# nicoloalbergoni/DeepLabV3Plus-Augmented-SuperResolution

Measured on AMD Instinct MI355X. Metric: augmented-copies/sec (fwd+realign+SR-iter) @512x512, higher is better.
Workload: dtype f32 (pointwise GEMMs: operands split into f16 hi+lo, hi*hi+hi*lo+lo*hi on f16 MFMA, f32 accumulate)

## Files before the change

__graft_entry__.py:

```python
from __future__ import annotations

import importlib.util
import os
import sys

ROOT = os.path.dirname(os.path.abspath(__file__))
if ROOT not in sys.path:
    sys.path.insert(0, ROOT)

PKG_DIR = os.path.join(ROOT, "deeplabv3plus-augmented-superresolution_amd")


def _load_build_module():
    spec = importlib.util.spec_from_file_location("asr_csrc_build", os.path.join(PKG_DIR, "csrc", "build.py"))
    mod = importlib.util.module_from_spec(spec)
    spec.loader.exec_module(mod)
    return mod


def build() -> None:
    lib = _load_build_module().build(force=False, verbose=True)
    assert os.path.exists(lib), lib
    import asr_amd
    asr_amd._lib.load()
    import asr_amd.ops
    print(f"built and loaded {lib} (ABI v{asr_amd._lib.load().asr_abi_version()})")


def smoke() -> None:
    import numpy as np
    import torch

    build()
    assert torch.cuda.is_available(), "smoke() needs a GPU"
    torch.cuda.set_device(0)
    dev = torch.device("cuda", 0)
    from asr_amd import ops, weights as W
    from asr_amd.model import DeeplabModel
    from asr_amd.pipeline import HotPath
    from asr_amd.superresolution_scripts.optimizer import Optimizer
    from asr_amd.superresolution_scripts.superresolution import Superresolution
    from asr_amd.superresolution_scripts.augmentation_utils import draw_augmentation_parameters
    from oracle import augment as o_aug, sr as o_sr
    from oracle.model import OracleDeeplabV3Plus

    size, feat, n_aug, iters, cls = (128, 128), (32, 32), 4, 5, 8
    weights = W.make_synthetic_weights(1234, 21)
    import bench
    img = bench.synth_image(np.random.default_rng(7), size[0])
    np.random.seed(1234)
    angles, shifts = draw_augmentation_parameters(n_aug, 0.15, 20)

    model = DeeplabModel(weights, size + (3,), 21, final_upsample=False, last_activation=None)
    img_dev = ops.to_device(img, device=dev)
    weights = bench.shifted_weights(weights, cls, bench.calibrate_class_bias(model, img_dev, cls))
# ... 41 lines not shown
```

deeplabv3plus-augmented-superresolution_amd/csrc/build.py:

```python
from __future__ import annotations

import os
import subprocess
import sys

HERE = os.path.dirname(os.path.abspath(__file__))
PKG = os.path.dirname(HERE)
LIB = os.path.join(PKG, "libasr_hip.so")
VARIANTS = {"phase": ["-DASR_GEMM_PHASE_PROFILE"],
            "diag": []}
VARIANT_SOURCES = {"diag": [(os.path.join("diag", "gemm_diag.hip"), [])]}

NO_PK_F32 = ["-Xclang", "-target-feature", "-Xclang", "-packed-fp32-ops"]
_HOST_NOISE = "'-packed-fp32-ops' is not a recognized feature for this target"

SOURCES = [
    ("core.cpp", []),
    ("warp.hip", ["-ffp-contract=off"] + NO_PK_F32),
    ("sr.hip", ["-ffp-contract=off"]),
    ("reduce.hip", ["-ffp-contract=off"] + NO_PK_F32),
    ("gemm.hip", ["-Wno-inline-asm"] + NO_PK_F32),
    ("dwconv.hip", NO_PK_F32),
    ("layers.hip", NO_PK_F32),
    ("sepconv.hip", NO_PK_F32),
# ... 31 lines not shown
    return any(os.path.getmtime(d) > t for d in deps)


def _postpass(hipcc, flags, src, obj, verbose):
    import importlib.util
    spec = importlib.util.spec_from_file_location("asr_pk_postpass", os.path.join(HERE, "pk_postpass.py"))
    pp = importlib.util.module_from_spec(spec)
    spec.loader.exec_module(pp)
    if not os.path.exists(os.path.join(pp.LLVM, "clang-offload-bundler")):
        print(f"build.py: no LLVM tools under {pp.LLVM}: {os.path.basename(src)} is built without packed-f32", file=sys.stderr, flush=True)
        return False
    try:
        n = pp.compile_with_postpass(hipcc, flags, src, obj)
    except pp.Unsafe as e:
        print(f"build.py: post-pass cannot split `{e}`: {os.path.basename(src)} is built without packed-f32", file=sys.stderr, flush=True)
        return False
    if verbose:
        print(f"{hipcc} ... {os.path.basename(src)} (packed-f32 post-pass: {n} op_sel:[0,1] instructions split)", flush=True)
    return True


def _isa_guard(lib):
    import importlib.util
    spec = importlib.util.spec_from_file_location("asr_isa_guard", os.path.join(HERE, "isa_guard.py"))
    guard = importlib.util.module_from_spec(spec)
    spec.loader.exec_module(guard)
    try:
        return guard.violations(lib)
    except guard.ToolMissing as e:
        print(f"build.py: isa_guard skipped ({e})", file=sys.stderr, flush=True)
        return []


def build(force=False, verbose=True):
    import fcntl
    variant = os.environ.get("ASR_BUILD_VARIANT", "")
    if variant and variant not in VARIANTS:
        raise ValueError(f"ASR_BUILD_VARIANT must be one of {sorted(VARIANTS)} (got {variant!r})")
    objdir = os.path.join(HERE, "build_" + variant if variant else "build")
    os.makedirs(objdir, exist_ok=True)
    with open(os.path.join(objdir, ".lock"), "w") as lock:
        fcntl.flock(lock, fcntl.LOCK_EX)
        try:
            return _build_locked(objdir, force, verbose, variant)
        finally:
            fcntl.flock(lock, fcntl.LOCK_UN)


def _build_locked(objdir, force, verbose, variant=""):
    hipcc = _hipcc()
    lib = os.path.join(PKG, f"libasr_hip_{variant}.so") if variant else LIB
    extra_all = VARIANTS.get(variant, []) + os.environ.get("ASR_EXTRA_HIPFLAGS", "").split()
    stamp = os.path.join(objdir, "flags.txt")
    flags_now = " ".join(COMMON + extra_all)
    if not os.path.exists(stamp) or open(stamp).read() != flags_now:
        force = True
    hdrs = [os.path.join(HERE, h) for h in HEADERS] + [os.path.abspath(__file__)]
    objs = []
    for src, extra in ALL_SOURCES + VARIANT_SOURCES.get(variant, []):
        s = os.path.join(HERE, src)
        o = os.path.join(objdir, os.path.splitext(os.path.basename(src))[0] + ".o")
        objs.append(o)
        if force or _stale(o, [s] + hdrs + ([os.path.join(HERE, "pk_postpass.py")] if src in POSTPASS else [])):
            if src in POSTPASS and _postpass(hipcc, COMMON + extra + extra_all, s, o, verbose):
                continue
            if src in POSTPASS:
                extra = extra + NO_PK_F32
            cmd = [hipcc] + COMMON + extra + extra_all + ["-c", s, "-o", o]
            if verbose:
                print(" ".join(cmd), flush=True)
            _compile(cmd)
    relinked = force or _stale(lib, objs)
    if relinked:
        cmd = [hipcc, "--offload-arch=gfx950", "-shared", "-fPIC", "-o", lib] + objs
        if verbose:
            print(" ".join(cmd), flush=True)
        subprocess.check_call(cmd)
    with open(stamp, "w") as fh:
        fh.write(flags_now)
    if relinked and not variant:
        bad = _isa_guard(lib)
        if bad:
            os.replace(lib, lib + ".rejected")
            raise RuntimeError("isa_guard: %d violation(s) in the product library, first: %s in %s (%s); kept as %s"
                               % (len(bad), bad[0][1], bad[0][0], bad[0][2], lib + ".rejected"))
    return lib


if __name__ == "__main__":
    print(build(force="--force" in sys.argv))
```

deeplabv3plus-augmented-superresolution_amd/csrc/diag/gemm_diag.hip:

```cpp
#include "../gemm_common.h"

namespace {


template <int PIECES_PER_LOADER = 16, bool MOCK_FUSED = false>
__global__ __launch_bounds__(768, 3) void pw_gemm_f16x3_pre_lw_kernel(PwArgs p) {
    constexpr int BM = 256, BN = 256, WN = 2, RT = 4, CT = 8;
    constexpr int A_BYTES = BM * 128, B_BYTES = 4 * BN * 16, STAGE_BYTES = A_BYTES + 2 * B_BYTES;
    constexpr int A_PIECES = A_BYTES / 1024;
    static_assert(4 * PIECES_PER_LOADER * 1024 == STAGE_BYTES, "four loader waves cover one stage");
    extern __shared__ __attribute__((aligned(16))) float smem[];
    char* const lds = reinterpret_cast<char*>(smem);

    const int nwg = gridDim.x, orig = blockIdx.x;
    const int q8 = nwg >> 3, r8 = nwg & 7, xcd = orig & 7;
    const int lid = (xcd < r8 ? xcd * (q8 + 1) : r8 * (q8 + 1) + (xcd - r8) * q8) + (orig >> 3);
    const int tile_m = lid / p.tiles_n, tile_n = lid % p.tiles_n;
    const int tid = threadIdx.x, lane = tid & 63, wave = __builtin_amdgcn_readfirstlane(tid >> 6);
    const int KT = p.Kpad / BK;

    if (MOCK_FUSED && wave >= 8) {
        const int w = wave - 8;
        const long long plane_bytes = (long long)p.Kpad * p.Npad * 2;
        const char* bsrc[8];
// ... 335 lines not shown
    a.taps = 1; a.cin = k; a.stride = 1; a.pad = 0; a.dil = 1;
    ASR_UNSUPPORTED(a.Npad % 256 != 0, "asr_diag_pwconv_presplit_8w: ceil128(n) must be a multiple of 256");
    a.tiles_n = (int)asr_cdiv(n, 256);
    const long long nwg = asr_cdiv(m, 256) * a.tiles_n;
    constexpr size_t lds = 2 * (256 * 128 + 2 * 4 * 256 * 16);
    auto kern8 = pw_gemm_f16x3_pre_kernel<4, 2, 2, 4>;
    static AsrDeviceOnce once;
    ASR_HIP_CHECK(asr_allow_dynamic_lds(once, reinterpret_cast<const void*>(kern8), (int)lds));
    hipLaunchKernelGGL(kern8, dim3((unsigned)nwg), dim3(512), lds, asr_stream(stream), a);
    ASR_LAUNCH_CHECK();
    return ASR_OK;
}

extern "C" int asr_diag_pwconv_presplit_lw(const void* x_split, const float* w_packed, const float* bias, const float* residual,
                                           float* y, int64_t m, int k, int n, int ldx_chunks, int ldy, int ldres, int relu,
                                           asr_stream_t stream) {
    ASR_REQUIRE(x_split && w_packed && y && m > 0 && k > 0 && n > 0, "asr_diag_pwconv_presplit_lw: bad arguments");
    PwArgs a{};
    a.x = reinterpret_cast<const float*>(x_split); a.wp = w_packed; a.bias = bias; a.res = residual; a.y = y;
    a.M = m; a.K = k; a.N = n; a.Npad = round_up(n, 128); a.Kpad = round_up(k, BK);
    a.ldx = ldx_chunks; a.ldy = ldy; a.ldres = ldres; a.relu = relu;
    a.taps = 1; a.cin = k; a.stride = 1; a.pad = 0; a.dil = 1;
    ASR_UNSUPPORTED(a.Npad % 256 != 0, "asr_diag_pwconv_presplit_lw: ceil128(n) must be a multiple of 256");
    a.tiles_n = (int)asr_cdiv(n, 256);
    const long long nwg = asr_cdiv(m, 256) * a.tiles_n;
    constexpr size_t lds = 2 * (256 * 128 + 2 * 4 * 256 * 16);
    auto kern = pw_gemm_f16x3_pre_lw_kernel<16, false>;
    static AsrDeviceOnce once;
    ASR_HIP_CHECK(asr_allow_dynamic_lds(once, reinterpret_cast<const void*>(kern), (int)lds));
    hipLaunchKernelGGL(kern, dim3((unsigned)nwg), dim3(768), lds, asr_stream(stream), a);
    ASR_LAUNCH_CHECK();
    return ASR_OK;
}
```

deeplabv3plus-augmented-superresolution_amd/csrc/gemm.hip:

```cpp
#include "gemm_common.h"

namespace {

__device__ __forceinline__ void xcd_tile(int id, int count, int tiles_n, int& tile_m, int& tile_n) {
    const int q8 = count >> 3, r8 = count & 7, xcd = id & 7;
    const int lid = (xcd < r8 ? xcd * (q8 + 1) : r8 * (q8 + 1) + (xcd - r8) * q8) + (id >> 3);
    tile_m = lid / tiles_n;
    tile_n = lid % tiles_n;
}

template <int WM, int WN, int TM, int TN, bool CONV>
__global__ __launch_bounds__(256) void pw_gemm_kernel(PwArgs p) {
    constexpr int BM = WM * TM * 32, BN = WN * TN * 32;
    constexpr int A_F4 = BM / 32;
    constexpr int B_F4 = BN / 32;
    extern __shared__ __attribute__((aligned(16))) float smem[];
    float* const sA = smem;
    float* const sB = smem + BM * BK;

    int tile_m, tile_n;
    xcd_tile(blockIdx.x, gridDim.x, p.tiles_n, tile_m, tile_n);

    const int tid = threadIdx.x;
    const int lane = tid & 63, wave = tid >> 6;
// ... 348 lines not shown
        base_b = reinterpret_cast<const char*>(p.wp) + (long long)tile_n * BN * 16;
#pragma unroll
        for (int j = 0; j < PIECES; ++j) {
            const int pi = first + j;
            {
                const int q = pi * 64 + lane, row = q >> 3, slot = (q & 7) ^ ((row >> 1) & 7);
                long long r = row;
                if (m0 + r >= p.M) r = p.M - 1 - m0;
                off_a[j] = (unsigned)(r * p.ldx * 128 + slot * 16);
            }
            {
                const int qb = pi * 64 + lane, plane = qb >> 10, r = qb & 1023, oct = r >> 8, col = r & 255;
                off_b[j] = (unsigned)(plane * plane_bytes + ((long long)oct * p.Npad + col) * 16);
            }
        }
    }
    __device__ __forceinline__ void issue_a(int kt, int slot) {
        char* const dst = lds + slot * UNIT + first * 1024;
        const char* const src = base_a + (long long)kt * 128;
#pragma unroll
        for (int j = 0; j < PIECES; ++j) glds16_sbase(src, off_a[j], dst + j * 1024);
    }
    __device__ __forceinline__ void issue_b(int kt, int slot) {
        char* const dst = lds + slot * UNIT + first * 1024;
        const char* const src = base_b + kt * kstep_b;
#pragma unroll
        for (int j = 0; j < PIECES; ++j) glds16_sbase(src, off_b[j], dst + j * 1024);
    }
    __device__ __forceinline__ void issue_bias(int tile_n, int slot) {
        if (p.bias && wave == 8) {
            int col = tile_n * BN + lane * 4;
            if (col + 3 >= p.N) col = 0;
            glds16_sbase(p.bias, (unsigned)col * 4u, lds + slot * UNIT);
        }
    }
};

template <class Mark>
__device__ __forceinline__ void mfma_tile(const PwArgs& p, f32x4 (&acc)[RT][CT], const char* lds, int& slot, int KT, int tile_n,
                                          int lane, int wm, int wn, Mark&& mark) {
    const int ct_valid = min(CT, max(0, (p.N - (tile_n * BN + wn * (CT * 16)) + 15) >> 4));
#pragma unroll
    for (int i = 0; i < RT; ++i)
#pragma unroll
        for (int j = 0; j < CT; ++j)
#pragma unroll
            for (int e = 0; e < 4; ++e) acc[i][j][e] = 0.f;

    auto kloop = [&](auto CTV_) {
        constexpr int CTV = decltype(CTV_)::value;
        for (int kt = 0; kt < KT; ++kt) {
            const int off_a = slot * UNIT, off_b = (slot + 1 >= RING ? 0 : slot + 1) * UNIT;
            slot = slot + 2 >= RING ? slot + 2 - RING : slot + 2;
            int ln = lane;
            asm volatile("" : "+v"(ln));
            const int l16 = ln & 15, oct = ln >> 4;
            const int swz = (l16 >> 1) & 7;
            const int a_row = off_a + (wm * RT * 16 + l16) * 128;
            const int a_hi = a_row + ((oct ^ swz) << 4), a_lo = a_row + (((4 + oct) ^ swz) << 4);
            const int b_col = off_b + (oct * BN + wn * CT * 16 + l16) * 16;
            f16x8 ah[2], al[2], bh[2], bl[2];
            auto read_a = [&](int half, int i) {
                ah[i] = *reinterpret_cast<const f16x8*>(lds + a_hi + (2 * half + i) * 2048);
                al[i] = *reinterpret_cast<const f16x8*>(lds + a_lo + (2 * half + i) * 2048);
            };
            auto read_b = [&](int j, int buf) {
// ... 36 lines not shown
}

}

__global__ __launch_bounds__(768, 3) ASR_PK_F32 void pw_gemm_f16x3_pre_ring_kernel(PwArgs p) {
    using namespace pre_ring;
    extern __shared__ __attribute__((aligned(16))) float smem[];
    char* const lds = reinterpret_cast<char*>(smem);

    int tile_m, tile_n;
    xcd_tile(blockIdx.x, gridDim.x, p.tiles_n, tile_m, tile_n);
    const int tid = threadIdx.x, lane = tid & 63, wave = __builtin_amdgcn_readfirstlane(tid >> 6);
    const int KT = p.Kpad / BK;

    if (wave >= 8) {
        Loader ldr(p, lds, wave, lane);
        ldr.setup(tile_m, tile_n);
        ldr.issue_a(0, 0);
        ldr.issue_b(0, 1);
        if (KT > 1) {
            ldr.issue_a(1, 2);
            asm volatile("s_waitcnt vmcnt(8)" ::: "memory");
        } else {
            asm volatile("s_waitcnt vmcnt(0)" ::: "memory");
        }
        __builtin_amdgcn_s_barrier();
#ifdef ASR_GEMM_PHASE_PROFILE
        long long ph[8] = {0, 0, 0, 0, 0, 0, 0, 0};
        long long tprev = (long long)__builtin_readcyclecounter();
#endif
        int slot_b = 3, slot_a = 4;
        const bool ep_fast = pw_ep_fast(p);
        const bool res_dma = ep_fast && p.res != nullptr;
        auto issue_res = [&](int rt, int slot_h0, int slot_h1) {
#pragma unroll
            for (int j = 0; j < 16; ++j) {
                const int r = (wave - 8) * 16 + j;
                long long m = (long long)tile_m * BM + (r >> 4) * 64 + rt * 16 + (r & 15);
                if (m >= p.M) m = p.M - 1;
                int col = tile_n * BN + ((lane ^ (r & 15)) << 2);
                if (col + 3 >= p.N) col = 0;
                glds16_sbase(p.res + m * p.ldres, (unsigned)col * 4u, lds + ((r >> 5) ? slot_h1 : slot_h0) * UNIT + (r & 31) * 1024);
            }
        };
        for (int kt = 0; kt < KT; ++kt) {
            if (kt + 1 < KT) ldr.issue_b(kt + 1, slot_b);
            if (kt + 2 < KT) {
                ldr.issue_a(kt + 2, slot_a);
                PHASE_MARK(0);
                asm volatile("s_waitcnt vmcnt(8)" ::: "memory");
            } else {
                if (kt + 1 == KT && ep_fast) {
                    ldr.issue_bias(tile_n, slot_a);
                    if (res_dma) issue_res(0, slot_b - 1 < 0 ? RING - 1 : slot_b - 1, slot_b);
                }
                PHASE_MARK(0);
                asm volatile("s_waitcnt vmcnt(0)" ::: "memory");
            }
            PHASE_MARK(1);
            __builtin_amdgcn_s_barrier();
            PHASE_MARK(2);
            if (kt + 1 < KT) {
                slot_b = slot_b + 2 >= RING ? slot_b + 2 - RING : slot_b + 2;
                slot_a = slot_a + 2 >= RING ? slot_a + 2 - RING : slot_a + 2;
            }
        }
        if (res_dma) {
            const int b0h0 = slot_b - 1 < 0 ? RING - 1 : slot_b - 1, b0h1 = slot_b;
            const int b1h0 = (slot_b + 2) % RING, b1h1 = (slot_b + 3) % RING;
#pragma unroll 1
            for (int rt = 1; rt < 4; ++rt) {
                if (rt & 1) issue_res(rt, b1h0, b1h1); else issue_res(rt, b0h0, b0h1);
                asm volatile("s_waitcnt vmcnt(0)" ::: "memory");
                __builtin_amdgcn_s_barrier();
            }
        }
#ifdef ASR_GEMM_PHASE_PROFILE
        if (tid == 512 && blockIdx.x < ASR_PHASE_BLOCKS)
            for (int i = 0; i < 3; ++i) g_phase_cycles[blockIdx.x * 16 + 8 + i] = ph[i];
#endif
        return;
    }

    const int wm = wave & 3, wn = wave >> 2;
    f32x4 acc[RT][CT];
#ifdef ASR_GEMM_PHASE_PROFILE
    long long ph[8] = {0, 0, 0, 0, 0, 0, 0, 0};
    long long tprev = (long long)__builtin_readcyclecounter();
#endif
    __builtin_amdgcn_s_barrier();
    PHASE_MARK(0);
#ifdef ASR_GEMM_PHASE_PROFILE
    const long long loop_c0 = (long long)__builtin_readcyclecounter(), loop_r0 = (long long)__builtin_amdgcn_s_memrealtime();
#endif
    int slot = 0;
    mfma_tile(p, acc, lds, slot, KT, tile_n, lane, wm, wn, [&](int i) { PHASE_MARK(i); });
#ifdef ASR_GEMM_PHASE_PROFILE
    if (tid == 0 && blockIdx.x < ASR_PHASE_BLOCKS) {
        g_phase_cycles[blockIdx.x * 16 + 11] = (long long)__builtin_readcyclecounter() - loop_c0;
        g_phase_cycles[blockIdx.x * 16 + 12] = (long long)__builtin_amdgcn_s_memrealtime() - loop_r0;
    }
#endif
    pw_epilogue16_ring<RT, CT>(p, acc, lds, slot, UNIT, RING, (long long)tile_m * BM + wm * (RT * 16), tile_n * BN + wn * (CT * 16),
                              wm, wn);
#ifdef ASR_GEMM_PHASE_PROFILE
// ... 47 lines not shown
                            asm volatile("s_waitcnt vmcnt(0)" ::: "memory");
                        }
                    } else {
                        asm volatile("s_waitcnt vmcnt(0)" ::: "memory");
                    }
                }
                __builtin_amdgcn_s_barrier();
                if (kt + 1 < KT) {
                    slot_b = slot_b + 2 >= RING ? slot_b + 2 - RING : slot_b + 2;
                    slot_a = slot_a + 2 >= RING ? slot_a + 2 - RING : slot_a + 2;
                }
            }
            asm volatile("s_waitcnt vmcnt(0)" ::: "memory");
            __builtin_amdgcn_s_barrier();
            s0 = ring(s0 + 2 * KT);
        }
        return;
    }

    const int wm = wave & 3, wn = wave >> 2;
    __builtin_amdgcn_s_barrier();
    int slot = 0;
    for (int t = wg; t < ntiles; t += G) {
        xcd_tile(t, ntiles, p.tiles_n, tile_m, tile_n);
        f32x4 acc[RT][CT];
        mfma_tile(p, acc, lds, slot, KT, tile_n, lane, wm, wn, [](int) {});
        pw_epilogue16_ring<RT, CT>(p, acc, lds, slot, UNIT, RING, (long long)tile_m * BM + wm * (RT * 16), tile_n * BN + wn * (CT * 16),
                                  wm, wn);
        asm volatile("s_waitcnt lgkmcnt(0)" ::: "memory");
        __builtin_amdgcn_s_barrier();
    }
}

__global__ __launch_bounds__(256) void pack_weights_f16x3_kernel(const float* __restrict__ w, _Float16* __restrict__ wp, int K,
                                                                 int N, int Kpad, int Npad) {
    const long long total = (long long)Kpad * Npad;
    for (long long o = (long long)blockIdx.x * 256 + threadIdx.x; o < total; o += (long long)gridDim.x * 256) {
        const int kr = (int)(o & 7);
        const long long t = o >> 3;
        const int n = (int)(t % Npad);
        const int k = (int)(t / Npad) * 8 + kr;
        const float v = (k < K && n < N) ? w[(long long)k * N + n] : 0.f;
        const _Float16 h = (_Float16)v;
        wp[o] = h;
        wp[total + o] = (_Float16)(v - (float)h);
    }
}

__global__ __launch_bounds__(256) void pack_weights_kernel(const float* __restrict__ w, float* __restrict__ wp, int K, int N,
                                                           int Kpad, int Npad) {
    const long long total = (long long)Kpad * Npad;
    for (long long o = (long long)blockIdx.x * 256 + threadIdx.x; o < total; o += (long long)gridDim.x * 256) {
        const int kr = (int)(o & 3);
        const long long t = o >> 2;
        const int n = (int)(t % Npad);
        const int k = (int)(t / Npad) * 4 + kr;
        wp[o] = (k < K && n < N) ? w[(long long)k * N + n] : 0.f;
    }
}

template <int WM, int WN, int TM, int TN, bool CONV>
int launch(const PwArgs& a, hipStream_t s) {
    constexpr int BM = WM * TM * 32, BN = WN * TN * 32;
    PwArgs p = a;
    p.tiles_n = (int)asr_cdiv(p.N, BN);
    const long long tiles_m = asr_cdiv(p.M, BM);
// ... 119 lines not shown
    ASR_HIP_CHECK(asr_allow_dynamic_lds(once, reinterpret_cast<const void*>(kern), (int)lds));
    hipLaunchKernelGGL(kern, dim3((unsigned)nwg), dim3(WM * WN * 64), lds, asr_stream(stream), a);
    ASR_LAUNCH_CHECK();
    return ASR_OK;
}

static int launch_f16x3(PwArgs a, int conv, asr_stream_t stream) {
    long long nwg = 0;
    const int rc = conv == 0 ? (a.N <= 64 ? launch_f16x3_shape<2, 2, 2, 1, false>(a, nwg, stream)
                                          : launch_f16x3_shape<2, 2, 2, 2, false>(a, nwg, stream))
                 : conv == 1 ? launch_f16x3_shape<2, 2, 2, 2, true>(a, nwg, stream)
                             : launch_f16x3_shape<2, 2, 2, 1, true>(a, nwg, stream);
    if (rc != ASR_OK) return rc;
#ifdef ASR_GEMM_PHASE_PROFILE
    {
        static long long host[ASR_PHASE_BLOCKS * 16];
        ASR_HIP_CHECK(hipDeviceSynchronize());
        ASR_HIP_CHECK(hipMemcpyFromSymbol(host, HIP_SYMBOL(g_phase_cycles), sizeof(host)));
        const long long nb = nwg < ASR_PHASE_BLOCKS ? nwg : ASR_PHASE_BLOCKS;
        double mean[16] = {0};
        for (long long b = 0; b < nb; ++b)
            for (int i = 0; i < 16; ++i) mean[i] += (double)host[b * 16 + i] / (double)nb;
        const int kt = (a.K + 31) / 32;
        const int ktm = kt > 1 ? kt - 1 : 1;
        fprintf(stderr, "[phase] M=%lld K=%d N=%d blocks=%lld ksteps=%d | prologue %.0f | per k-step: issue %.0f  lds+mfma %.0f  vmwait %.0f  "
                        "barrier1 %.0f  split+store %.0f  barrier2 %.0f | epilogue %.0f | block total %.0f cycles\n",
                (long long)a.M, a.K, a.N, nwg, kt, mean[0], mean[1] / kt, mean[2] / kt, mean[3] / ktm, mean[4] / ktm, mean[5] / ktm,
                mean[6] / ktm, mean[7], mean[0] + mean[1] + mean[2] + mean[3] + mean[4] + mean[5] + mean[6] + mean[7]);
    }
#endif
    return ASR_OK;
}

extern "C" int asr_pwconv_mfma_f16x3(const float* x, const float* w_packed, const float* bias, const float* residual, float* y,
                                     int64_t m, int k, int n, int ldx, int ldy, int ldres, int relu, int sub_stride,
                                     int h_in, int w_in, asr_stream_t stream) {
    int rc = check_common("asr_pwconv_mfma_f16x3", x, w_packed, y, m, k, n, ldx, ldy, residual, ldres);
    if (rc != ASR_OK) return rc;
    ASR_REQUIRE(ldx >= k, "asr_pwconv_mfma_f16x3: ldx < k");
    ASR_UNSUPPORTED(k & 3, "asr_pwconv_mfma_f16x3: k must be a multiple of 4 (got %d)", k);
    PwArgs a{};
    a.x = x; a.wp = w_packed; a.bias = bias; a.res = residual; a.y = y;
    a.M = m; a.K = k; a.N = n; a.Npad = round_up(n, 128); a.Kpad = round_up(k, BK);
    a.ldx = ldx; a.ldy = ldy; a.ldres = ldres; a.relu = relu;
    a.taps = 1; a.cin = k; a.stride = 1; a.pad = 0; a.dil = 1;
    if (sub_stride > 1) {
        ASR_REQUIRE(h_in > 0 && w_in > 0, "asr_pwconv_mfma_f16x3: h_in/w_in required with sub_stride");
        a.h_in = h_in; a.w_in = w_in; a.stride = sub_stride;
        a.h_out = (h_in + sub_stride - 1) / sub_stride;
        a.w_out = (w_in + sub_stride - 1) / sub_stride;
        ASR_REQUIRE(m % ((long long)a.h_out * a.w_out) == 0, "asr_pwconv_mfma_f16x3: m is not a whole number of %dx%d maps",
                    a.h_out, a.w_out);
    }
    return launch_f16x3(a, 0, stream);
}

extern "C" int asr_pwconv_mfma_f16x3_presplit(const void* x_split, const float* w_packed, const float* bias,
                                              const float* residual, float* y, int64_t m, int k, int n, int ldx_chunks, int ldy,
                                              int ldres, int relu, asr_stream_t stream) {
    ASR_REQUIRE(x_split && w_packed && y, "asr_pwconv_mfma_f16x3_presplit: null pointer");
    ASR_REQUIRE(m > 0 && k > 0 && n > 0, "asr_pwconv_mfma_f16x3_presplit: bad shape m=%lld k=%d n=%d", (long long)m, k, n);
    ASR_REQUIRE(ldy >= n && (!residual || ldres >= n), "asr_pwconv_mfma_f16x3_presplit: ldy / ldres < n");
    PwArgs a{};
    a.x = reinterpret_cast<const float*>(x_split); a.wp = w_packed; a.bias = bias; a.res = residual; a.y = y;
    a.M = m; a.K = k; a.N = n; a.Npad = round_up(n, 128); a.Kpad = round_up(k, BK);
    a.ldx = ldx_chunks; a.ldy = ldy; a.ldres = ldres; a.relu = relu;
    a.taps = 1; a.cin = k; a.stride = 1; a.pad = 0; a.dil = 1;
    ASR_REQUIRE(ldx_chunks * BK >= a.Kpad, "asr_pwconv_mfma_f16x3_presplit: ldx_chunks * 32 < ceil32(k)");
    ASR_UNSUPPORTED(a.Npad % 256 != 0, "asr_pwconv_mfma_f16x3_presplit: ceil128(n) must be a multiple of 256 (n=%d)", n);
    ASR_UNSUPPORTED(reinterpret_cast<uintptr_t>(x_split) & 127, "asr_pwconv_mfma_f16x3_presplit: x_split must be 128-byte aligned");
    ASR_UNSUPPORTED((long long)ldx_chunks * 128 * 256 >= (1LL << 32) || (long long)a.Kpad * a.Npad * 4 + (long long)a.Npad * 64 >= (1LL << 32),
                    "asr_pwconv_mfma_f16x3_presplit: operands too large for 32-bit tile offsets (k=%d n=%d ldx_chunks=%d)", k, n, ldx_chunks);
    constexpr int bm = 256, bn = 256;
    a.tiles_n = (int)asr_cdiv(n, bn);
    const long long nwg = asr_cdiv(m, bm) * a.tiles_n;
    ASR_REQUIRE(nwg <= 0x7fffffffLL, "asr_pwconv_mfma_f16x3_presplit: grid too large");
    constexpr size_t lds = 5 * 32 * 1024;
    const int cus = asr_device_cu_count();
    ASR_REQUIRE(cus > 0, "asr_pwconv_mfma_f16x3_presplit: no device");
    const int cu_count = cus >= 8 ? cus / 8 * 8 : cus;
    if (!residual && a.Kpad / BK >= 4 && nwg > cu_count) {
        auto kern = pw_gemm_f16x3_pre_ring_persist_kernel;
        static AsrDeviceOnce once;
        ASR_HIP_CHECK(asr_allow_dynamic_lds(once, reinterpret_cast<const void*>(kern), (int)lds));
        hipLaunchKernelGGL(kern, dim3((unsigned)cu_count), dim3(768), lds, asr_stream(stream), a, (int)nwg);
        ASR_LAUNCH_CHECK();
        return ASR_OK;
// ... 45 lines not shown
```

deeplabv3plus-augmented-superresolution_amd/csrc/gemm_common.h:

```cpp
#pragma once
#include "asr_common.h"
#include <utility>

typedef float f32x16 __attribute__((ext_vector_type(16)));
typedef float f32x4 __attribute__((ext_vector_type(4)));
typedef _Float16 f16x8 __attribute__((ext_vector_type(8)));

namespace {

constexpr int BK = 32;

struct PwArgs {
    const float* x;
    const float* wp;
    const float* bias;
    const float* res;
    float* y;
    long long M;
    int K, N, Npad, Kpad;
    int ldx, ldy, ldres;
    int relu;
    int tiles_n;
    int taps;
    int cin;
    int h_in, w_in, h_out, w_out, stride, pad, dil;
};

template <int WM, int WN, int TM, int TN, bool RES_AHEAD = false>
__device__ __forceinline__ void pw_epilogue(const PwArgs& p, f32x16 (&acc)[TM][TN], float* smem, int tile_m, int tile_n,
                                            int wave, int lane) {
    constexpr int BM = WM * TM * 32, BN = WN * TN * 32;
    constexpr int WCOLS = TN * 32;
    constexpr int LPR = WCOLS / 4;
    constexpr int RPI = 64 / LPR;
    const int wm = wave / WN, wn = wave % WN;
    const int l32 = lane & 31, hh = lane >> 5;
    float* const stage = smem + wave * (32 * WCOLS);
    const bool vec_ok = ((p.N & 3) == 0) && ((p.ldy & 3) == 0) && ((reinterpret_cast<uintptr_t>(p.y) & 15) == 0) &&
                        (!p.res || (((p.ldres & 3) == 0) && ((reinterpret_cast<uintptr_t>(p.res) & 15) == 0)));
// ... 101 lines not shown
            __builtin_amdgcn_sched_barrier(0);
#pragma unroll
            for (int q = 0; q < RES_DEPTH; ++q) request(q);
        }
#pragma unroll
        for (int q = 0; q < NQ; ++q) {
            const int r = q * RPI + r_in;
            const long long m = m_base + r;
            f32x4 v = *reinterpret_cast<const f32x4*>(stage + r * WCOLS + c4 * 4);
            f32x4 rq = {0.f, 0.f, 0.f, 0.f};
            if (res_vec) {
                rq = rv[q % RES_DEPTH];
                if (q + RES_DEPTH < NQ) request(q + RES_DEPTH);
            }
            if (m < p.M && n < p.N) {
                if (vec_ok) {
                    if (p.res) v += rq;
                    *reinterpret_cast<f32x4*>(p.y + m * p.ldy + n) = v;
                } else {
#pragma unroll
                    for (int t = 0; t < 4; ++t)
                        if (n + t < p.N) {
                            float o = v[t];
                            if (p.res) o += p.res[m * p.ldres + n + t];
                            p.y[m * p.ldy + n + t] = o;
                        }
                }
            }
        }
    }
}


__device__ __forceinline__ bool pw_ep_fast(const PwArgs& p) {
    return ((p.N & 3) == 0) && ((p.ldy & 3) == 0) && ((reinterpret_cast<uintptr_t>(p.y) & 15) == 0) &&
           ((reinterpret_cast<uintptr_t>(p.bias) & 15) == 0) &&
           (!p.res || (((p.ldres & 3) == 0) && ((reinterpret_cast<uintptr_t>(p.res) & 15) == 0)));
}

template <int RT, int CT>
__device__ __forceinline__ void pw_epilogue16_ring(const PwArgs& p, f32x4 (&acc)[RT][CT], const char* lds, int f, int unit, int ring,
                                                   long long m_wave, int n_wave, int wm, int wn) {
    int lane;
    {
        int z = 0;
        asm volatile("" : "+v"(z));
        lane = (int)__builtin_amdgcn_mbcnt_hi(~0u, __builtin_amdgcn_mbcnt_lo(~0u, (unsigned)z));
    }
    const int l16 = lane & 15, q4 = lane >> 4;
    const bool fast = pw_ep_fast(p);
    const bool res_dma = fast && p.res != nullptr;
    const bool rows_ok = m_wave + RT * 16 <= p.M;
    auto slot_of = [&](int k) { const int v = f + k; return v >= ring ? v - ring : v; };
    const int n0 = n_wave + 4 * q4;
    if (fast && rows_ok) {
        const char* const bias_lds = lds + slot_of(2) * unit + (wn * (CT * 16) + 4 * q4) * 4;
        const unsigned yoff = ((unsigned)l16 * (unsigned)p.ldy + (unsigned)n0) * 4u;
        const int relu = p.relu;
        const bool has_bias = p.bias != nullptr;
#pragma unroll
        for (int rt = 0; rt < RT; ++rt) {
            char* const yrow = reinterpret_cast<char*>(p.y + (m_wave + rt * 16) * p.ldy);
            const int r = wm * 16 + l16;
            const char* const res_lds = lds + slot_of((rt & 1) * 3 + (r >> 5)) * unit + (r & 31) * 1024;
            const int s0 = wn * (CT * 4) + q4;
#pragma unroll
            for (int ct = 0; ct < CT; ++ct) {
// ... 91 lines not shown
```

deeplabv3plus-augmented-superresolution_amd/csrc/isa_guard.py:

```python
from __future__ import annotations

import os
import re
import struct
import subprocess
import sys
import tempfile

HERE = os.path.dirname(os.path.abspath(__file__))
PKG = os.path.dirname(HERE)
_MAGIC = b"__CLANG_OFFLOAD_BUNDLE__"
_LLVM_BIN = [os.environ.get("ASR_LLVM_BIN", ""), "/opt/rocm/lib/llvm/bin", "/opt/rocm/llvm/bin"]

MODE_WRITERS = ("entry_stem_fused_kernel", "conv3x3_stem_mfma_kernel", "pw_gemm_f16x3_kernel", "sepconv_fused_kernel",
                "dw_stream_full_kernel", "aspp_dw3_phase_kernel")
PK_KERNELS = ("dw_stream_full_kernel", "pw_gemm_f16x3_pre_ring", "sepconv_fused_kernel", "entry_stem_fused_kernel",
              "conv3x3_stem_kernel", "conv3x3_stem_mfma_kernel",
              "sr_")

_PK_F32 = re.compile(r"\bv_pk_(mul|add|fma)_f32\b")
_SGPR_SRC = re.compile(r"(?<![a-z_0-9])(s\[\d+:\d+\]|(s\d+|vcc|exec|ttmp\d+|ttmp\[\d+:\d+\]|m0)\b)")
_OP_SEL = re.compile(r"\bop_sel:\[([01,]+)\]")


def erratum_form(inst):
    if not _PK_F32.search(inst):
        return False
    m = _OP_SEL.search(inst)
    if not m:
        return False
    sel = [int(v) for v in m.group(1).split(",")]
    if len(sel) < 2 or sel[0] != 0 or sel[1] != 1:
        return False
    ops = inst.split(None, 1)[1].split(",")
    return len(ops) >= 3 and ops[2].strip().startswith("v[")


class ToolMissing(RuntimeError):
    """llvm-objcopy / llvm-objdump / llvm-readelf of the ROCm LLVM are not installed where this runs."""


def _tool(name):
    for d in _LLVM_BIN:
        p = os.path.join(d, name)
        if d and os.path.exists(p):
            return p
    raise ToolMissing(f"{name} not found (set ASR_LLVM_BIN)")
# ... 117 lines not shown
```

Baseline: 2223.

## Add f32-A ring GEMM kernel that splits activations in loader waves

```diff
diff --git a/__graft_entry__.py b/__graft_entry__.py
--- a/__graft_entry__.py
+++ b/__graft_entry__.py
@@ -19,8 +19,11 @@
 
 
 def build() -> None:
-    lib = _load_build_module().build(force=False, verbose=True)
+    builder = _load_build_module()
+    lib = builder.build(force=False, verbose=True)
     assert os.path.exists(lib), lib
+    diag = builder.build(force=False, verbose=True, variant="diag")
+    assert os.path.exists(diag), diag
     import asr_amd
     asr_amd._lib.load()
     import asr_amd.ops
diff --git a/deeplabv3plus-augmented-superresolution_amd/csrc/build.py b/deeplabv3plus-augmented-superresolution_amd/csrc/build.py
--- a/deeplabv3plus-augmented-superresolution_amd/csrc/build.py
+++ b/deeplabv3plus-augmented-superresolution_amd/csrc/build.py
@@ -87,9 +87,10 @@
         return []
 
 
-def build(force=False, verbose=True):
+def build(force=False, verbose=True, variant=None):
     import fcntl
-    variant = os.environ.get("ASR_BUILD_VARIANT", "")
+    if variant is None:
+        variant = os.environ.get("ASR_BUILD_VARIANT", "")
     if variant and variant not in VARIANTS:
         raise ValueError(f"ASR_BUILD_VARIANT must be one of {sorted(VARIANTS)} (got {variant!r})")
     objdir = os.path.join(HERE, "build_" + variant if variant else "build")
@@ -112,9 +113,16 @@
         force = True
     hdrs = [os.path.join(HERE, h) for h in HEADERS] + [os.path.abspath(__file__)]
     objs = []
+    shared = os.path.join(HERE, "build") if variant and not VARIANTS[variant] and not os.environ.get("ASR_EXTRA_HIPFLAGS") else None
+    if shared:
+        build(False, verbose, variant="")
     for src, extra in ALL_SOURCES + VARIANT_SOURCES.get(variant, []):
         s = os.path.join(HERE, src)
-        o = os.path.join(objdir, os.path.splitext(os.path.basename(src))[0] + ".o")
+        own = shared is None or (src, extra) in VARIANT_SOURCES.get(variant, [])
+        o = os.path.join(objdir if own else shared, os.path.splitext(os.path.basename(src))[0] + ".o")
+        if not own:
+            objs.append(o)
+            continue
         objs.append(o)
         if force or _stale(o, [s] + hdrs + ([os.path.join(HERE, "pk_postpass.py")] if src in POSTPASS else [])):
             if src in POSTPASS and _postpass(hipcc, COMMON + extra + extra_all, s, o, verbose):
diff --git a/deeplabv3plus-augmented-superresolution_amd/csrc/diag/gemm_diag.hip b/deeplabv3plus-augmented-superresolution_amd/csrc/diag/gemm_diag.hip
--- a/deeplabv3plus-augmented-superresolution_amd/csrc/diag/gemm_diag.hip
+++ b/deeplabv3plus-augmented-superresolution_amd/csrc/diag/gemm_diag.hip
@@ -391,3 +391,10 @@
     ASR_LAUNCH_CHECK();
     return ASR_OK;
 }
+
+extern "C" int asr_diag_pwconv_f16x3_routed(const float* x, const float* w_packed, const float* bias, const float* residual,
+                                            float* y, int64_t m, int k, int n, int ldx, int ldy, int ldres, int relu,
+                                            int sub_stride, int h_in, int w_in, asr_stream_t stream, int route, int* taken) {
+    return asr_pwconv_f16x3_routed(x, w_packed, bias, residual, y, m, k, n, ldx, ldy, ldres, relu, sub_stride, h_in, w_in, stream,
+                                   route, taken);
+}
diff --git a/deeplabv3plus-augmented-superresolution_amd/csrc/gemm.hip b/deeplabv3plus-augmented-superresolution_amd/csrc/gemm.hip
--- a/deeplabv3plus-augmented-superresolution_amd/csrc/gemm.hip
+++ b/deeplabv3plus-augmented-superresolution_amd/csrc/gemm.hip
@@ -404,6 +404,17 @@
             int col = tile_n * BN + lane * 4;
             if (col + 3 >= p.N) col = 0;
             glds16_sbase(p.bias, (unsigned)col * 4u, lds + slot * UNIT);
+        }
+    }
+    __device__ __forceinline__ void issue_res(int tile_m, int tile_n, int rt, int slot_h0, int slot_h1) {
+#pragma unroll
+        for (int j = 0; j < 16; ++j) {
+            const int r = (wave - 8) * 16 + j;
+            long long m = (long long)tile_m * BM + (r >> 4) * 64 + rt * 16 + (r & 15);
+            if (m >= p.M) m = p.M - 1;
+            int col = tile_n * BN + ((lane ^ (r & 15)) << 2);
+            if (col + 3 >= p.N) col = 0;
+            glds16_sbase(p.res + m * p.ldres, (unsigned)col * 4u, lds + ((r >> 5) ? slot_h1 : slot_h0) * UNIT + (r & 31) * 1024);
         }
     }
 };
@@ -506,17 +517,6 @@
         int slot_b = 3, slot_a = 4;
         const bool ep_fast = pw_ep_fast(p);
         const bool res_dma = ep_fast && p.res != nullptr;
-        auto issue_res = [&](int rt, int slot_h0, int slot_h1) {
-#pragma unroll
-            for (int j = 0; j < 16; ++j) {
-                const int r = (wave - 8) * 16 + j;
-                long long m = (long long)tile_m * BM + (r >> 4) * 64 + rt * 16 + (r & 15);
-                if (m >= p.M) m = p.M - 1;
-                int col = tile_n * BN + ((lane ^ (r & 15)) << 2);
-                if (col + 3 >= p.N) col = 0;
-                glds16_sbase(p.res + m * p.ldres, (unsigned)col * 4u, lds + ((r >> 5) ? slot_h1 : slot_h0) * UNIT + (r & 31) * 1024);
-            }
-        };
         for (int kt = 0; kt < KT; ++kt) {
             if (kt + 1 < KT) ldr.issue_b(kt + 1, slot_b);
             if (kt + 2 < KT) {
@@ -526,7 +526,7 @@
             } else {
                 if (kt + 1 == KT && ep_fast) {
                     ldr.issue_bias(tile_n, slot_a);
-                    if (res_dma) issue_res(0, slot_b - 1 < 0 ? RING - 1 : slot_b - 1, slot_b);
+                    if (res_dma) ldr.issue_res(tile_m, tile_n, 0, slot_b - 1 < 0 ? RING - 1 : slot_b - 1, slot_b);
                 }
                 PHASE_MARK(0);
                 asm volatile("s_waitcnt vmcnt(0)" ::: "memory");
@@ -544,7 +544,7 @@
             const int b1h0 = (slot_b + 2) % RING, b1h1 = (slot_b + 3) % RING;
 #pragma unroll 1
             for (int rt = 1; rt < 4; ++rt) {
-                if (rt & 1) issue_res(rt, b1h0, b1h1); else issue_res(rt, b0h0, b0h1);
+                if (rt & 1) ldr.issue_res(tile_m, tile_n, rt, b1h0, b1h1); else ldr.issue_res(tile_m, tile_n, rt, b0h0, b0h1);
                 asm volatile("s_waitcnt vmcnt(0)" ::: "memory");
                 __builtin_amdgcn_s_barrier();
             }
@@ -658,6 +658,209 @@
     }
 }
 
+namespace pre_ring {
+
+#define ASR_A_CLOBBERS \
+    "v104", "v105", "v106", "v107", "v108", "v109", "v110", "v111", "v112", "v113", "v114", "v115", "v116", "v117", "v118", "v119", \
+    "v120", "v121", "v122", "v123", "v124", "v125", "v126", "v127", "v128", "v129", "v130", "v131", "v132", "v133", "v134", "v135", \
+    "v136", "v137", "v138", "v139", "v140", "v141", "v142", "v143", "v144", "v145", "v146", "v147", "v148", "v149", "v150", "v151", \
+    "v152", "v153", "v154", "v155", "v156", "v157", "v158", "v159", "v160", "v161", "v162", "v163", "v164", "v165", "v166", "v167"
+#define ASR_A_REQUEST_SET0 \
+    "global_load_dwordx4 v[104:107], %0, %8\n\t" "global_load_dwordx4 v[108:111], %1, %8\n\t" \
+    "global_load_dwordx4 v[112:115], %2, %8\n\t" "global_load_dwordx4 v[116:119], %3, %8\n\t" \
+    "global_load_dwordx4 v[120:123], %4, %8\n\t" "global_load_dwordx4 v[124:127], %5, %8\n\t" \
+    "global_load_dwordx4 v[128:131], %6, %8\n\t" "global_load_dwordx4 v[132:135], %7, %8"
+#define ASR_A_REQUEST_SET1 \
+    "global_load_dwordx4 v[136:139], %0, %8\n\t" "global_load_dwordx4 v[140:143], %1, %8\n\t" \
+    "global_load_dwordx4 v[144:147], %2, %8\n\t" "global_load_dwordx4 v[148:151], %3, %8\n\t" \
+    "global_load_dwordx4 v[152:155], %4, %8\n\t" "global_load_dwordx4 v[156:159], %5, %8\n\t" \
+    "global_load_dwordx4 v[160:163], %6, %8\n\t" "global_load_dwordx4 v[164:167], %7, %8"
+#define ASR_A_TAKE_SET0 \
+    "v_mov_b64 %0, v[104:105]\n\t" "v_mov_b64 %1, v[106:107]\n\t" "v_mov_b64 %2, v[108:109]\n\t" "v_mov_b64 %3, v[110:111]\n\t" \
+    "v_mov_b64 %4, v[112:113]\n\t" "v_mov_b64 %5, v[114:115]\n\t" "v_mov_b64 %6, v[116:117]\n\t" "v_mov_b64 %7, v[118:119]\n\t" \
+    "v_mov_b64 %8, v[120:121]\n\t" "v_mov_b64 %9, v[122:123]\n\t" "v_mov_b64 %10, v[124:125]\n\t" "v_mov_b64 %11, v[126:127]\n\t" \
+    "v_mov_b64 %12, v[128:129]\n\t" "v_mov_b64 %13, v[130:131]\n\t" "v_mov_b64 %14, v[132:133]\n\t" "v_mov_b64 %15, v[134:135]"
+#define ASR_A_TAKE_SET1 \
+    "v_mov_b64 %0, v[136:137]\n\t" "v_mov_b64 %1, v[138:139]\n\t" "v_mov_b64 %2, v[140:141]\n\t" "v_mov_b64 %3, v[142:143]\n\t" \
+    "v_mov_b64 %4, v[144:145]\n\t" "v_mov_b64 %5, v[146:147]\n\t" "v_mov_b64 %6, v[148:149]\n\t" "v_mov_b64 %7, v[150:151]\n\t" \
+    "v_mov_b64 %8, v[152:153]\n\t" "v_mov_b64 %9, v[154:155]\n\t" "v_mov_b64 %10, v[156:157]\n\t" "v_mov_b64 %11, v[158:159]\n\t" \
+    "v_mov_b64 %12, v[160:161]\n\t" "v_mov_b64 %13, v[162:163]\n\t" "v_mov_b64 %14, v[164:165]\n\t" "v_mov_b64 %15, v[166:167]"
+#define ASR_A_REQUEST(text, src, o)                                                                                        \
+    asm volatile(text : : "v"(o[0]), "v"(o[1]), "v"(o[2]), "v"(o[3]), "v"(o[4]), "v"(o[5]), "v"(o[6]), "v"(o[7]), "s"(src)   \
+                 : "memory", ASR_A_CLOBBERS)
+#define ASR_A_TAKE(n, text, d)                                                                                             \
+    asm volatile("s_waitcnt vmcnt(" #n ")\n\t" text                                                                        \
+                 : "=v"(d[0]), "=v"(d[1]), "=v"(d[2]), "=v"(d[3]), "=v"(d[4]), "=v"(d[5]), "=v"(d[6]), "=v"(d[7]), "=v"(d[8]),  \
+                   "=v"(d[9]), "=v"(d[10]), "=v"(d[11]), "=v"(d[12]), "=v"(d[13]), "=v"(d[14]), "=v"(d[15])                  \
+                 :                                                                                                         \
+                 : "memory", ASR_A_CLOBBERS)
+
+constexpr int A_PAIRS = 4;
+
+struct F32ALoader {
+    const PwArgs& p;
+    char* const lds;
+    const int lw, lane, oct, KT;
+    unsigned off[A_PAIRS];
+    bool row_ok[A_PAIRS];
+    bool ragged;
+    unsigned lds_hi;
+    const char* base;
+
+    __device__ __forceinline__ F32ALoader(const PwArgs& p_, char* lds_, int wave_, int lane_, int KT_)
+        : p(p_), lds(lds_), lw(wave_ - 8), lane(lane_), oct(lane_ & 3), KT(KT_) {}
+
+    __device__ __forceinline__ void setup(int tile_m) {
+        const long long m0 = (long long)tile_m * BM;
+        base = reinterpret_cast<const char*>(p.x) + m0 * p.ldx * 4;
+        ragged = m0 + BM > p.M;
+        const int row_in = ((lane >> 2) & 1) * 8 + (lane >> 3);
+        lds_hi = (unsigned)((lw * 64 + row_in) * 128 + ((oct ^ ((row_in >> 1) & 7)) << 4));
+#pragma unroll
+        for (int j = 0; j < A_PAIRS; ++j) {
+            long long r = (lw * A_PAIRS + j) * 16 + row_in;
+            row_ok[j] = m0 + r < p.M;
+            if (!row_ok[j]) r = p.M - 1 - m0;
+            off[j] = (unsigned)((r * p.ldx + oct * 8) * 4);
+        }
+    }
+    __device__ __forceinline__ bool tail(int kt) const { return kt + 1 == KT && p.K < p.Kpad; }
+
+    template <int SET>
+    __device__ __forceinline__ void request(int kt) {
+        const char* const src = base + (long long)kt * 128;
+        const int k = kt * BK + oct * 8;
+        const unsigned d0 = (unsigned)(4 * (min(k, p.K - 4) - k)), d1 = (unsigned)(4 * (min(k + 4, p.K - 4) - k));
+        unsigned o[2 * A_PAIRS];
+#pragma unroll
+        for (int j = 0; j < A_PAIRS; ++j) {
+            o[2 * j] = off[j] + d0;
+            o[2 * j + 1] = off[j] + d1;
+        }
+        if constexpr (SET == 0) ASR_A_REQUEST(ASR_A_REQUEST_SET0, src, o);
+        else ASR_A_REQUEST(ASR_A_REQUEST_SET1, src, o);
+    }
+    template <int SET, int YOUNGER>
+    __device__ __forceinline__ void take_and_store(int kt, int slot) {
+        static_assert((SET == 0 || SET == 1) && (YOUNGER == 8 || YOUNGER == 16), "register set / wait count");
+        asr_f32x2 d[4 * A_PAIRS];
+        if constexpr (SET == 0 && YOUNGER == 16) ASR_A_TAKE(16, ASR_A_TAKE_SET0, d);
+        if constexpr (SET == 0 && YOUNGER == 8) ASR_A_TAKE(8, ASR_A_TAKE_SET0, d);
+        if constexpr (SET == 1 && YOUNGER == 16) ASR_A_TAKE(16, ASR_A_TAKE_SET1, d);
+        if constexpr (SET == 1 && YOUNGER == 8) ASR_A_TAKE(8, ASR_A_TAKE_SET1, d);
+        f32x4 R[2 * A_PAIRS];
+#pragma unroll
+        for (int i = 0; i < 2 * A_PAIRS; ++i) R[i] = f32x4{d[2 * i].x, d[2 * i].y, d[2 * i + 1].x, d[2 * i + 1].y};
+        store(kt, slot, R);
+    }
+    __device__ __forceinline__ void store(int kt, int slot, f32x4 (&R)[2 * A_PAIRS]) {
+        const f32x4 zero4 = {0.f, 0.f, 0.f, 0.f};
+        if (tail(kt) || ragged) {
+            const int k = kt * BK + oct * 8;
+            const bool k0_ok = k < p.K, k1_ok = k + 4 < p.K;
+#pragma unroll
+            for (int j = 0; j < A_PAIRS; ++j) {
+                R[2 * j] = (row_ok[j] && k0_ok) ? R[2 * j] : zero4;
+                R[2 * j + 1] = (row_ok[j] && k1_ok) ? R[2 * j + 1] : zero4;
+            }
+        }
+        char* const unit = lds + slot * UNIT;
+#pragma unroll
+        for (int j = 0; j < A_PAIRS; ++j) {
+            f16x8 hi, lo;
+            split_f16x8(R[2 * j], R[2 * j + 1], hi, lo);
+            *reinterpret_cast<f16x8*>(unit + (lds_hi + j * 2048)) = hi;
+            *reinterpret_cast<f16x8*>(unit + ((lds_hi ^ 64u) + j * 2048)) = lo;
+        }
+    }
+};
+
+}
+
+__global__ __launch_bounds__(768, 3) void pw_gemm_f16x3_f32a_ring_kernel(PwArgs p) {
+    using namespace pre_ring;
+    extern __shared__ __attribute__((aligned(16))) float smem[];
+    char* const lds = reinterpret_cast<char*>(smem);
+
+    int tile_m, tile_n;
+    xcd_tile(blockIdx.x, gridDim.x, p.tiles_n, tile_m, tile_n);
+    const int tid = threadIdx.x, lane = tid & 63, wave = __builtin_amdgcn_readfirstlane(tid >> 6);
+    const int KT = p.Kpad / BK;
+
+    if (wave >= 8) {
+        asr_enable_f16_saturation();
+        Loader ldr(p, lds, wave, lane);
+        ldr.setup(tile_m, tile_n);
+        F32ALoader fa(p, lds, wave, lane, KT);
+        fa.setup(tile_m);
+        fa.request<0>(0);
+        ldr.issue_b(0, 1);
+        if (KT > 1) {
+            fa.request<1>(1);
+            fa.take_and_store<0, 16>(0, 0);
+            asm volatile("s_waitcnt vmcnt(8)" ::: "memory");
+        } else {
+            fa.take_and_store<0, 8>(0, 0);
+            asm volatile("s_waitcnt vmcnt(0)" ::: "memory");
+        }
+        asm volatile("s_waitcnt lgkmcnt(0)" ::: "memory");
+        __builtin_amdgcn_s_barrier();
+
+        int slot_b = 3, slot_a = 4;
+        const bool ep_fast = pw_ep_fast(p);
+        const bool res_dma = ep_fast && p.res != nullptr;
+        auto kstep = [&](int kt, auto NEXT_) {
+            constexpr int NEXT = decltype(NEXT_)::value, CUR = 1 - NEXT;
+            if (kt + 2 < KT) {
+                ldr.issue_b(kt + 1, slot_b);
+                fa.request<NEXT>(kt + 2);
+                fa.take_and_store<CUR, 16>(kt + 1, slot_b - 1 < 0 ? RING - 1 : slot_b - 1);
+                asm volatile("s_waitcnt vmcnt(8)" ::: "memory");
+                asm volatile("s_waitcnt lgkmcnt(0)" ::: "memory");
+            } else if (kt + 1 < KT) {
+                ldr.issue_b(kt + 1, slot_b);
+                fa.take_and_store<CUR, 8>(kt + 1, slot_b - 1 < 0 ? RING - 1 : slot_b - 1);
+                asm volatile("s_waitcnt vmcnt(0)" ::: "memory");
+                asm volatile("s_waitcnt lgkmcnt(0)" ::: "memory");
+            } else {
+                if (ep_fast) {
+                    ldr.issue_bias(tile_n, slot_a);
+                    if (res_dma) ldr.issue_res(tile_m, tile_n, 0, slot_b - 1 < 0 ? RING - 1 : slot_b - 1, slot_b);
+                }
+                asm volatile("s_waitcnt vmcnt(0)" ::: "memory");
+            }
+            __builtin_amdgcn_s_barrier();
+            if (kt + 1 < KT) {
+                slot_b = slot_b + 2 >= RING ? slot_b + 2 - RING : slot_b + 2;
+                slot_a = slot_a + 2 >= RING ? slot_a + 2 - RING : slot_a + 2;
+            }
+        };
+        for (int kt = 0; kt < KT; kt += 2) {
+            kstep(kt, std::integral_constant<int, 0>{});
+            if (kt + 1 < KT) kstep(kt + 1, std::integral_constant<int, 1>{});
+        }
+        if (res_dma) {
+            const int b0h0 = slot_b - 1 < 0 ? RING - 1 : slot_b - 1, b0h1 = slot_b;
+            const int b1h0 = (slot_b + 2) % RING, b1h1 = (slot_b + 3) % RING;
+#pragma unroll 1
+            for (int rt = 1; rt < 4; ++rt) {
+                if (rt & 1) ldr.issue_res(tile_m, tile_n, rt, b1h0, b1h1); else ldr.issue_res(tile_m, tile_n, rt, b0h0, b0h1);
+                asm volatile("s_waitcnt vmcnt(0)" ::: "memory");
+                __builtin_amdgcn_s_barrier();
+            }
+        }
+        return;
+    }
+
+    const int wm = wave & 3, wn = wave >> 2;
+    f32x4 acc[RT][CT];
+    __builtin_amdgcn_s_barrier();
+    int slot = 0;
+    mfma_tile(p, acc, lds, slot, KT, tile_n, lane, wm, wn, [](int) {});
+    pw_epilogue16_ring<RT, CT>(p, acc, lds, slot, UNIT, RING, (long long)tile_m * BM + wm * (RT * 16), tile_n * BN + wn * (CT * 16),
+                              wm, wn);
+}
+
 __global__ __launch_bounds__(256) void pack_weights_f16x3_kernel(const float* __restrict__ w, _Float16* __restrict__ wp, int K,
                                                                  int N, int Kpad, int Npad) {
     const long long total = (long long)Kpad * Npad;
@@ -843,9 +1046,30 @@
     return ASR_OK;
 }
 
-extern "C" int asr_pwconv_mfma_f16x3(const float* x, const float* w_packed, const float* bias, const float* residual, float* y,
-                                     int64_t m, int k, int n, int ldx, int ldy, int ldres, int relu, int sub_stride,
-                                     int h_in, int w_in, asr_stream_t stream) {
+static bool f32a_ring_can_run(const PwArgs& a) {
+    return a.stride == 1 && a.h_out == 0 && a.Npad % 256 == 0 && a.M >= 256 && pw_ep_fast(a) &&
+           (long long)a.ldx * 4 * 256 + (long long)a.Kpad * 4 < (1LL << 32) &&
+           (long long)a.Kpad * a.Npad * 4 + (long long)a.Npad * 64 < (1LL << 32);
+}
+constexpr int kF32aRingMinK = 256;
+
+static int launch_f32a_ring(PwArgs a, asr_stream_t stream) {
+    constexpr int bm = 256, bn = 256;
+    a.tiles_n = (int)asr_cdiv(a.N, bn);
+    const long long nwg = asr_cdiv(a.M, bm) * a.tiles_n;
+    ASR_REQUIRE(nwg <= 0x7fffffffLL, "asr_pwconv_mfma_f16x3: grid too large");
+    constexpr size_t lds = 5 * 32 * 1024;
+    auto kern = pw_gemm_f16x3_f32a_ring_kernel;
+    static AsrDeviceOnce once;
+    ASR_HIP_CHECK(asr_allow_dynamic_lds(once, reinterpret_cast<const void*>(kern), (int)lds));
+    hipLaunchKernelGGL(kern, dim3((unsigned)nwg), dim3(768), lds, asr_stream(stream), a);
+    ASR_LAUNCH_CHECK();
+    return ASR_OK;
+}
+
+int asr_pwconv_f16x3_routed(const float* x, const float* w_packed, const float* bias, const float* residual, float* y, int64_t m,
+                            int k, int n, int ldx, int ldy, int ldres, int relu, int sub_stride, int h_in, int w_in,
+                            asr_stream_t stream, int route, int* taken) {
     int rc = check_common("asr_pwconv_mfma_f16x3", x, w_packed, y, m, k, n, ldx, ldy, residual, ldres);
     if (rc != ASR_OK) return rc;
     ASR_REQUIRE(ldx >= k, "asr_pwconv_mfma_f16x3: ldx < k");
@@ -863,7 +1087,22 @@
         ASR_REQUIRE(m % ((long long)a.h_out * a.w_out) == 0, "asr_pwconv_mfma_f16x3: m is not a whole number of %dx%d maps",
                     a.h_out, a.w_out);
     }
-    return launch_f16x3(a, 0, stream);
+    ASR_REQUIRE(route >= ASR_PW_ROUTE_AUTO && route <= ASR_PW_ROUTE_QUERY, "asr_pwconv_mfma_f16x3: unknown route %d", route);
+    const bool can = f32a_ring_can_run(a);
+    ASR_UNSUPPORTED(route == ASR_PW_ROUTE_RING && !can,
+                    "asr_pwconv_mfma_f16x3: the ring kernel cannot take this launch (m=%lld k=%d n=%d ldx=%d ldy=%d sub_stride=%d)",
+                    (long long)m, k, n, ldx, ldy, sub_stride);
+    const bool ring = route == ASR_PW_ROUTE_RING || (route != ASR_PW_ROUTE_SPLIT && can && k >= kF32aRingMinK);
+    if (taken) *taken = ring ? ASR_PW_ROUTE_RING : ASR_PW_ROUTE_SPLIT;
+    if (route == ASR_PW_ROUTE_QUERY) return ASR_OK;
+    return ring ? launch_f32a_ring(a, stream) : launch_f16x3(a, 0, stream);
+}
+
+extern "C" int asr_pwconv_mfma_f16x3(const float* x, const float* w_packed, const float* bias, const float* residual, float* y,
+                                     int64_t m, int k, int n, int ldx, int ldy, int ldres, int relu, int sub_stride,
+                                     int h_in, int w_in, asr_stream_t stream) {
+    return asr_pwconv_f16x3_routed(x, w_packed, bias, residual, y, m, k, n, ldx, ldy, ldres, relu, sub_stride, h_in, w_in, stream,
+                                   ASR_PW_ROUTE_AUTO, nullptr);
 }
 
 extern "C" int asr_pwconv_mfma_f16x3_presplit(const void* x_split, const float* w_packed, const float* bias,
diff --git a/deeplabv3plus-augmented-superresolution_amd/csrc/gemm_common.h b/deeplabv3plus-augmented-superresolution_amd/csrc/gemm_common.h
--- a/deeplabv3plus-augmented-superresolution_amd/csrc/gemm_common.h
+++ b/deeplabv3plus-augmented-superresolution_amd/csrc/gemm_common.h
@@ -5,6 +5,12 @@
 typedef float f32x16 __attribute__((ext_vector_type(16)));
 typedef float f32x4 __attribute__((ext_vector_type(4)));
 typedef _Float16 f16x8 __attribute__((ext_vector_type(8)));
+
+enum { ASR_PW_ROUTE_AUTO = 0, ASR_PW_ROUTE_SPLIT = 1, ASR_PW_ROUTE_RING = 2, ASR_PW_ROUTE_QUERY = 3 };
+__attribute__((visibility("hidden"))) int asr_pwconv_f16x3_routed(const float* x, const float* w_packed, const float* bias,
+                                                                  const float* residual, float* y, int64_t m, int k, int n,
+                                                                  int ldx, int ldy, int ldres, int relu, int sub_stride, int h_in,
+                                                                  int w_in, asr_stream_t stream, int route, int* taken);
 
 namespace {
 
@@ -172,7 +178,7 @@
 }
 
 
-__device__ __forceinline__ bool pw_ep_fast(const PwArgs& p) {
+__host__ __device__ __forceinline__ bool pw_ep_fast(const PwArgs& p) {
     return ((p.N & 3) == 0) && ((p.ldy & 3) == 0) && ((reinterpret_cast<uintptr_t>(p.y) & 15) == 0) &&
            ((reinterpret_cast<uintptr_t>(p.bias) & 15) == 0) &&
            (!p.res || (((p.ldres & 3) == 0) && ((reinterpret_cast<uintptr_t>(p.res) & 15) == 0)));
diff --git a/deeplabv3plus-augmented-superresolution_amd/csrc/isa_guard.py b/deeplabv3plus-augmented-superresolution_amd/csrc/isa_guard.py
--- a/deeplabv3plus-augmented-superresolution_amd/csrc/isa_guard.py
+++ b/deeplabv3plus-augmented-superresolution_amd/csrc/isa_guard.py
@@ -12,7 +12,7 @@
 _MAGIC = b"__CLANG_OFFLOAD_BUNDLE__"
 _LLVM_BIN = [os.environ.get("ASR_LLVM_BIN", ""), "/opt/rocm/lib/llvm/bin", "/opt/rocm/llvm/bin"]
 
-MODE_WRITERS = ("entry_stem_fused_kernel", "conv3x3_stem_mfma_kernel", "pw_gemm_f16x3_kernel", "sepconv_fused_kernel",
+MODE_WRITERS = ("entry_stem_fused_kernel", "conv3x3_stem_mfma_kernel", "pw_gemm_f16x3_kernel", "pw_gemm_f16x3_f32a_ring_kernel", "sepconv_fused_kernel",
                 "dw_stream_full_kernel", "aspp_dw3_phase_kernel")
 PK_KERNELS = ("dw_stream_full_kernel", "pw_gemm_f16x3_pre_ring", "sepconv_fused_kernel", "entry_stem_fused_kernel",
               "conv3x3_stem_kernel", "conv3x3_stem_mfma_kernel",
```

Result: no change. 2236 (median of 6 runs) (+0.6%).
